# williamleif/GraphSAGE

Measured on NVIDIA H100. Metric: seed_nodes_per_sec, higher is better.
Workload: dtype f32

## Files before the change

### graphsage_b200/csrc/maxpool_tc.cu

```cuda
#include "tc_common.cuh"

namespace gs {

constexpr int MP_KCOLS = 64;
constexpr int MP_IMG = 128 * 128;
constexpr int MP_MAX_KB = 10;
constexpr int MP_STAGES = 3;
constexpr int MP_THREADS = 256;

struct MpParams {
  const __nv_bfloat16* table;
  int64_t n_rows, pitch;
  int32_t K, kblocks;
  const int32_t* row_ids;
  int64_t row0;
  int64_t n_groups;
  int32_t k, G;
  int32_t n_slices;
  const unsigned char* wimg;
  const float* bias;
  int32_t pool_mean;
  float* out;
  int64_t ldo;
  const float* dhp;
  int64_t lddhp;
  unsigned char* dp;
  float* dbm_part;
};

__global__ void __launch_bounds__(256) maxpool_pack_kernel(const float* __restrict__ W, int64_t ldw, int K, int hidden,
                                                           int kblocks, unsigned char* __restrict__ img) {
  const int slice = blockIdx.x / kblocks, kb = blockIdx.x % kblocks;
  unsigned char* dst = img + ((int64_t)slice * kblocks + kb) * MP_IMG;
  for (int q = threadIdx.x; q < 128 * 8; q += blockDim.x) {
    const int c = q >> 7, n = q & 127;
    const int gn = slice * 128 + n, k0 = kb * MP_KCOLS + c * 8;
    __nv_bfloat162 h[4];
#pragma unroll
    for (int e = 0; e < 4; ++e) {
      float a = (gn < hidden && k0 + 2 * e < K) ? W[(int64_t)(k0 + 2 * e) * ldw + gn] : 0.f;
      float b = (gn < hidden && k0 + 2 * e + 1 < K) ? W[(int64_t)(k0 + 2 * e + 1) * ldw + gn] : 0.f;
      h[e] = __floats2bfloat162_rn(a, b);
    }
    *reinterpret_cast<uint4*>(dst + sw128_off(n, c)) = *reinterpret_cast<uint4*>(h);
  }
}

template <bool kRowsA, int NT, int DEPTH, int PROD, bool kGrad = false>
__global__ void __launch_bounds__(MP_THREADS, NT == 128 ? 2 : 1) maxpool_mlp_kernel(const __grid_constant__ MpParams prm) {
  constexpr int ROWS_IMG = NT * 128;
  constexpr int STAGE = ROWS_IMG + MP_IMG;
  constexpr int CPT = NT / 32;
  constexpr int LOOK = MP_STAGES - DEPTH;
  constexpr int MI = kRowsA ? NT / 128 : 1;
  constexpr int NI = kRowsA ? 1 : NT / 128;
  constexpr int LD = NT + 1;
  static_assert(128 * LD * 4 <= MP_STAGES * STAGE, "epilogue staging must fit in the operand ring");
  static_assert(LOOK >= 1, "at least one K-block of prefetch");
  extern __shared__ unsigned char smem_raw[];
  __shared__ __align__(8) uint64_t full_b[MP_STAGES];
  unsigned char* smem = reinterpret_cast<unsigned char*>((reinterpret_cast<uintptr_t>(smem_raw) + 1023) & ~(uintptr_t)1023);
  const int tid = threadIdx.x, wg = tid >> 7, lane = tid & 31, wq = (tid >> 5) & 3;
  const int slice = blockIdx.x % prm.n_slices;
  const int64_t t = blockIdx.x / prm.n_slices;
  const int kblocks = prm.kblocks;

  if (tid == 0) {
    for (int s = 0; s < MP_STAGES; ++s) mbar_init(&full_b[s], 1);
    fence_mbar_init();
  }
  __syncthreads();

  const int c = tid & 7, r0 = tid >> 3;
  const int rows_valid = prm.G * prm.k;
  const __nv_bfloat16* rowp[CPT];
#pragma unroll
  for (int i = 0; i < CPT; ++i) {
    const int r = r0 + 32 * i;
    const int64_t flat = t * rows_valid + r;
    rowp[i] = nullptr;
    if (r < rows_valid && flat < prm.n_groups * prm.k) {
      int64_t id = prm.row_ids ? (int64_t)prm.row_ids[flat] : prm.row0 + flat;
      if (id < 0 || id >= prm.n_rows) id = prm.n_rows - 1;
      rowp[i] = prm.table + id * prm.pitch;
    }
  }
  const unsigned char* wsrc = prm.wimg + (int64_t)slice * kblocks * MP_IMG;
  auto stage_of = [&](int kb) { return smem + (size_t)(kb % MP_STAGES) * STAGE; };
  auto issue = [&](int kb) {
    if (kb < kblocks) {
      unsigned char* st = stage_of(kb);
      if (tid == 0) {
        mbar_expect_tx(&full_b[kb % MP_STAGES], MP_IMG);
        bulk_g2s(st + ROWS_IMG, wsrc + (int64_t)kb * MP_IMG, MP_IMG, &full_b[kb % MP_STAGES]);
      }
      if constexpr (PROD == 0) {
        const int col = kb * MP_KCOLS + c * 8;
#pragma unroll
        for (int i = 0; i < CPT; ++i) {
          int nbytes = 0;
          if (rowp[i] != nullptr && col < prm.K) nbytes = min(8, prm.K - col) * 2;
          const void* src = nbytes ? (const void*)(rowp[i] + col) : (const void*)prm.table;
          cp_async16(st + sw128_off(r0 + 32 * i, c), src, nbytes);
        }
      }
    }
    if constexpr (PROD == 0) cp_async_commit();
  };
  uint4 regs[PROD == 1 ? CPT : 1];
  auto load_regs = [&](int kb) {
    const int col = kb * MP_KCOLS + c * 8;
#pragma unroll
    for (int i = 0; i < CPT; ++i) {
      regs[i] = make_uint4(0, 0, 0, 0);
      if (rowp[i] == nullptr || col >= prm.K) continue;
      if (col + 8 <= prm.K) {
        regs[i] = __ldg(reinterpret_cast<const uint4*>(rowp[i] + col));
      } else {
        unsigned short h[8] = {0, 0, 0, 0, 0, 0, 0, 0};
        const unsigned short* src = reinterpret_cast<const unsigned short*>(rowp[i] + col);
        for (int e = 0; e < prm.K - col; ++e) h[e] = __ldg(src + e);
        regs[i] = *reinterpret_cast<const uint4*>(h);
      }
    }
  };

  for (int j = 0; j < LOOK; ++j) issue(j);
  if constexpr (PROD == 1) load_regs(0);
  float acc[MI * NI][64];
#pragma unroll
  for (int a = 0; a < MI * NI; ++a)
#pragma unroll
    for (int i = 0; i < 64; ++i) acc[a][i] = 0.f;
  for (int kb = 0; kb < kblocks; ++kb) {
    unsigned char* st = stage_of(kb);
    if constexpr (PROD == 0) {
      cp_async_wait<LOOK - 1>();
    } else {
#pragma unroll
      for (int i = 0; i < CPT; ++i) *reinterpret_cast<uint4*>(st + sw128_off(r0 + 32 * i, c)) = regs[i];
    }
    fence_proxy_async();
    __syncthreads();
    issue(kb + LOOK);
    if constexpr (PROD == 1) {
      if (kb + 1 < kblocks) load_regs(kb + 1);
    }
    mbar_wait(&full_b[kb % MP_STAGES], (uint32_t)(kb / MP_STAGES) & 1u);
    const uint32_t rows_s = smem_u32(st), w_s = smem_u32(st + ROWS_IMG);
#pragma unroll
    for (int a = 0; a < MI * NI; ++a) acc_fence(acc[a]);
    wgmma_fence();
#pragma unroll
    for (int k = 0; k < 4; ++k)
#pragma unroll
      for (int mi = 0; mi < MI; ++mi)
#pragma unroll
        for (int ni = 0; ni < NI; ++ni) {
          const uint64_t adesc = kRowsA ? make_smem_desc(rows_s + (uint32_t)((wg * (NT / 2) + mi * 64) * 128))
                                        : make_smem_desc(w_s + (uint32_t)(wg * 64 * 128));
          const uint64_t bdesc = kRowsA ? make_smem_desc(w_s) : make_smem_desc(rows_s + (uint32_t)(ni * 128 * 128));
          wgmma_m64n128<true>(acc[mi * NI + ni], adesc + (uint64_t)(k * 2), bdesc + (uint64_t)(k * 2),
                              (kb > 0 || k > 0) ? 1u : 0u);
        }
    wgmma_commit();
    wgmma_wait<DEPTH - 1>();
#pragma unroll
    for (int a = 0; a < MI * NI; ++a) acc_fence(acc[a]);
  }
  wgmma_wait<0>();
#pragma unroll
  for (int a = 0; a < MI * NI; ++a) acc_fence(acc[a]);
  if constexpr (PROD == 0) cp_async_wait<0>();
  __syncthreads();

  float* stage = reinterpret_cast<float*>(smem);
#pragma unroll
  for (int mi = 0; mi < MI; ++mi)
#pragma unroll
    for (int ni = 0; ni < NI; ++ni)
#pragma unroll
      for (int j = 0; j < 16; ++j)
#pragma unroll
        for (int e = 0; e < 4; ++e) {
          const int m = wq * 16 + (lane >> 2) + 8 * (e >> 1);
          const int n = 8 * j + 2 * (lane & 3) + (e & 1);
          const int row = kRowsA ? wg * (NT / 2) + mi * 64 + m : ni * 128 + n;
          const int col = kRowsA ? n : wg * 64 + m;
          stage[col * LD + row] = acc[mi * NI + ni][4 * j + e];
        }
  __syncthreads();
  const int k = prm.k, G = prm.G;
  if constexpr (kGrad) {
    static_assert(kRowsA && NT == 128, "B1 reads the <rows as A, 128-row tile> staging layout");
    const int cc = tid & (TC_BN - 1), hcol = slice * 128 + cc;
    const float b = prm.bias ? prm.bias[hcol] : 0.f;
    float part = 0.f;
    for (int g = tid >> 7; g < G; g += 2) {
      const int64_t gg = t * G + g;
      if (gg >= prm.n_groups) break;
      float* p = stage + cc * LD + g * k;
      const float d = prm.dhp[gg * prm.lddhp + hcol];
      float s = 0.f;
      if (prm.pool_mean) {
        const float q = d / (float)k;
        for (int j = 0; j < k; ++j) {
          const float v = (p[j] + b > 0.f) ? q : 0.f;
          p[j] = v;
          s += v;
        }
      } else {
        float m = -3.0e38f;
        for (int j = 0; j < k; ++j) m = fmaxf(m, p[j]);
        const float hp = fmaxf(m + b, 0.f);
        int cnt = 0;
        if (hp > 0.f)
          for (int j = 0; j < k; ++j) cnt += (p[j] + b == hp) ? 1 : 0;
        const float q = cnt ? d / (float)cnt : 0.f;
        for (int j = 0; j < k; ++j) {
          const float v = (cnt && p[j] + b == hp) ? q : 0.f;
          p[j] = v;
          s += v;
        }
      }
      part += s;
    }
    float* red = stage + TC_BN * LD;
    red[(tid >> 7) * TC_BN + cc] = part;
    __syncthreads();
    if (tid < TC_BN) prm.dbm_part[t * (int64_t)prm.n_slices * 128 + hcol] = red[cc] + red[TC_BN + cc];
    const int nvalid = (int)min((int64_t)G * k, prm.n_groups * k - t * (int64_t)G * k);
    unsigned char* img = prm.dp + (t * prm.n_slices + slice) * (int64_t)(2 * MP_IMG);
#pragma unroll
    for (int i = 0; i < (2 * 128 * 8) / MP_THREADS; ++i) {
      const int q = tid + MP_THREADS * i;
      const int h = q >> 10, n = (q >> 3) & 127, c = q & 7;
      const int r0 = h * 64 + c * 8;
      __nv_bfloat162 v[4];
#pragma unroll
      for (int e = 0; e < 4; ++e) {
        const float a0 = (r0 + 2 * e < nvalid) ? stage[n * LD + r0 + 2 * e] : 0.f;
        const float a1 = (r0 + 2 * e + 1 < nvalid) ? stage[n * LD + r0 + 2 * e + 1] : 0.f;
        v[e] = __floats2bfloat162_rn(a0, a1);
      }
      *reinterpret_cast<uint4*>(img + h * MP_IMG + sw128_off(n, c)) = *reinterpret_cast<uint4*>(v);
    }
  } else {
    for (int u = tid; u < TC_BN * G; u += MP_THREADS) {
      const int cc = u & (TC_BN - 1), g = u / TC_BN;
      const int64_t gg = t * G + g;
      if (gg >= prm.n_groups) break;
      const float* p = stage + cc * LD + g * k;
      const int hcol = slice * 128 + cc;
      const float b = prm.bias ? prm.bias[hcol] : 0.f;
      float res;
      if (prm.pool_mean) {
        float sacc = 0.f;
        for (int j = 0; j < k; ++j) sacc += fmaxf(p[j] + b, 0.f);
        res = sacc / (float)k;
      } else {
        float m = -3.0e38f;
        int j = 0;
        for (; j + 8 <= k; j += 8) {
          float v[8];
#pragma unroll
          for (int w = 0; w < 8; ++w) v[w] = p[j + w];
          m = fmaxf(m, fmaxf(fmaxf(fmaxf(v[0], v[1]), fmaxf(v[2], v[3])), fmaxf(fmaxf(v[4], v[5]), fmaxf(v[6], v[7]))));
        }
        for (; j < k; ++j) m = fmaxf(m, p[j]);
        res = fmaxf(m + b, 0.f);
      }
      prm.out[gg * prm.ldo + hcol] = res;
    }
  }
}

template <bool kRowsA, int NT, int DEPTH, int PROD>
static int32_t launch_k4(const MpParams& prm, int64_t n_tiles, int cluster, cudaStream_t st) {
  const void* fn = (const void*)maxpool_mlp_kernel<kRowsA, NT, DEPTH, PROD>;
  const int smem = MP_STAGES * (NT * 128 + MP_IMG) + 1024;
  const int32_t rc_attr = ensure_dyn_smem(fn, smem);
  if (rc_attr != GS_OK) return rc_attr;
  cudaLaunchConfig_t cfg;
  memset(&cfg, 0, sizeof(cfg));
  cfg.gridDim = dim3((unsigned)(n_tiles * prm.n_slices));
  cfg.blockDim = dim3((unsigned)MP_THREADS);
  cfg.dynamicSmemBytes = smem;
  cfg.stream = st;
  cudaLaunchAttribute attr;
  if (cluster > 1) {
    attr.id = cudaLaunchAttributeClusterDimension;
    attr.val.clusterDim.x = (unsigned)cluster;
    attr.val.clusterDim.y = 1;
    attr.val.clusterDim.z = 1;
    cfg.attrs = &attr;
    cfg.numAttrs = 1;
  }
  MpParams p = prm;
  void* args[1] = {(void*)&p};
  GS_CUDA(cudaLaunchKernelExC(&cfg, fn, args));
  return launch_check("maxpool_mlp_kernel");
}

template <bool kRowsA, int NT>
static int32_t launch_k4_by(const MpParams& prm, int64_t n_tiles, int cluster, int depth, int producer, cudaStream_t st) {
  if (depth == 2)
    return producer == 1 ? launch_k4<kRowsA, NT, 2, 1>(prm, n_tiles, cluster, st) : launch_k4<kRowsA, NT, 2, 0>(prm, n_tiles, cluster, st);
  return producer == 1 ? launch_k4<kRowsA, NT, 1, 1>(prm, n_tiles, cluster, st) : launch_k4<kRowsA, NT, 1, 0>(prm, n_tiles, cluster, st);
}

}

extern "C" {

int64_t gs_maxpool_mlp_workspace_bytes(int32_t K, int32_t hidden) {
  if (K < 1 || hidden < 1) return -1;
  const int kblocks = (K + gs::MP_KCOLS - 1) / gs::MP_KCOLS, slices = (hidden + 127) / 128;
  return (int64_t)kblocks * slices * gs::MP_IMG;
}

int32_t gs_maxpool_mlp_pack(const float* Wm, int64_t ldw, int32_t K, int32_t hidden, void* workspace, void* stream) {
  GS_REQUIRE(Wm && workspace && K >= 1 && hidden >= 1 && ldw >= hidden, "gs_maxpool_mlp_pack: bad arguments");
  GS_REQUIRE((reinterpret_cast<uintptr_t>(workspace) & 127u) == 0, "gs_maxpool_mlp_pack: workspace must be 128-byte aligned");
  const int kblocks = (K + gs::MP_KCOLS - 1) / gs::MP_KCOLS, slices = (hidden + 127) / 128;
  gs::maxpool_pack_kernel<<<kblocks * slices, 256, 0, (cudaStream_t)stream>>>(Wm, ldw, K, hidden, kblocks,
                                                                             (unsigned char*)workspace);
  return gs::launch_check("maxpool_pack_kernel");
}

static int32_t pool_mlp_fused(const void* table_bf16, int64_t n_rows, int32_t K, int64_t pitch, const int32_t* row_ids,
                              int64_t row0, int64_t n_groups, int32_t k, const void* packed_weights, const float* bias,
                              int32_t hidden, float* out, int64_t ldo, int32_t pool_mean, void* stream) {
  GS_REQUIRE(n_groups >= 0 && k >= 1, "gs_maxpool_mlp_fused: bad n_groups / k");
  if (n_groups == 0) return GS_OK;
  GS_REQUIRE(table_bf16 && packed_weights && out, "gs_maxpool_mlp_fused: NULL pointer");
  GS_REQUIRE(n_rows > 0 && n_rows < 0x7fffffffLL && K >= 1 && pitch >= K, "gs_maxpool_mlp_fused: bad table shape");
  GS_REQUIRE((pitch * 2) % 16 == 0 && (reinterpret_cast<uintptr_t>(table_bf16) & 15u) == 0,
             "gs_maxpool_mlp_fused: table rows must be 16-byte multiples and 16-byte aligned (pitch %% 8 == 0)");
  GS_REQUIRE((reinterpret_cast<uintptr_t>(packed_weights) & 127u) == 0, "gs_maxpool_mlp_fused: packed weights misaligned");
  const int nt = gs::tuning("k4_tile", 128) == 256 ? 256 : 128;
  if (k > nt || (K + gs::MP_KCOLS - 1) / gs::MP_KCOLS > gs::MP_MAX_KB || hidden % 128 != 0) {
    gs::set_error("gs_maxpool_mlp_fused: needs k <= %d, K <= %d, hidden %% 128 == 0 (k=%d K=%d hidden=%d)", nt,
                  gs::MP_MAX_KB * gs::MP_KCOLS, k, K, hidden);
    return GS_ERR_UNSUPPORTED;
  }
  GS_REQUIRE(ldo >= hidden, "gs_maxpool_mlp_fused: ldo < hidden");
  gs::MpParams prm;
  memset(&prm, 0, sizeof(prm));
  prm.table = (const __nv_bfloat16*)table_bf16;
  prm.n_rows = n_rows; prm.pitch = pitch; prm.K = K; prm.kblocks = (K + gs::MP_KCOLS - 1) / gs::MP_KCOLS;
  prm.row_ids = row_ids; prm.row0 = row0; prm.n_groups = n_groups; prm.k = k; prm.G = nt / k;
  prm.n_slices = hidden / 128;
  prm.wimg = (const unsigned char*)packed_weights; prm.bias = bias; prm.out = out; prm.ldo = ldo;
  prm.pool_mean = pool_mean;
  const int64_t n_tiles = (n_groups + prm.G - 1) / prm.G;
  GS_REQUIRE(n_tiles * prm.n_slices < 0x7fffffffLL, "gs_maxpool_mlp_fused: too many groups (%lld)", (long long)n_groups);
  int cluster = gs::tuning("k4_cluster", 0);
  if (cluster < 0 || cluster > prm.n_slices) cluster = prm.n_slices;
  while (cluster > 1 && (cluster > 8 || prm.n_slices % cluster != 0)) --cluster;
  const int depth = gs::tuning("k4_mma_depth", 1) == 2 ? 2 : 1;
  const int producer = gs::tuning("k4_producer", 0) == 1 ? 1 : 0;
  const bool rows_a = gs::tuning("k4_operands", 1) != 0;
  const cudaStream_t st = (cudaStream_t)stream;
  if (rows_a)
    return nt == 256 ? gs::launch_k4_by<true, 256>(prm, n_tiles, cluster, depth, producer, st)
                     : gs::launch_k4_by<true, 128>(prm, n_tiles, cluster, depth, producer, st);
  return nt == 256 ? gs::launch_k4_by<false, 256>(prm, n_tiles, cluster, depth, producer, st)
                   : gs::launch_k4_by<false, 128>(prm, n_tiles, cluster, depth, producer, st);
}

int32_t gs_maxpool_mlp_fused(const void* table_bf16, int64_t n_rows, int32_t K, int64_t pitch, const int32_t* row_ids,
                             int64_t row0, int64_t n_groups, int32_t k, const void* packed_weights, const float* bias,
                             int32_t hidden, float* out, int64_t ldo, void* stream) {
  return pool_mlp_fused(table_bf16, n_rows, K, pitch, row_ids, row0, n_groups, k, packed_weights, bias, hidden, out, ldo, 0,
                        stream);
}

int32_t gs_meanpool_mlp_fused(const void* table_bf16, int64_t n_rows, int32_t K, int64_t pitch, const int32_t* row_ids,
                              int64_t row0, int64_t n_groups, int32_t k, const void* packed_weights, const float* bias,
                              int32_t hidden, float* out, int64_t ldo, void* stream) {
  return pool_mlp_fused(table_bf16, n_rows, K, pitch, row_ids, row0, n_groups, k, packed_weights, bias, hidden, out, ldo, 1,
                        stream);
}

int64_t gs_pool_mlp_dp_bytes(int64_t n_groups, int32_t k, int32_t hidden) {
  if (n_groups < 0 || k < 1 || k > 128 || hidden < 128 || hidden % 128 != 0) return -1;
  const int64_t G = 128 / k, n_tiles = (n_groups + G - 1) / G;
  return n_tiles * hidden * (256 + 4);
}

int32_t gs_pool_mlp_backward_dp(const void* table_bf16, int64_t n_rows, int32_t K, int64_t pitch, const int32_t* row_ids,
                                int64_t row0, int64_t n_groups, int32_t k, const void* packed_weights, const float* bias,
                                int32_t hidden, const float* dhp, int64_t lddhp, int32_t pool_mean, void* dp, void* stream) {
  GS_REQUIRE(n_groups >= 0 && k >= 1, "gs_pool_mlp_backward_dp: bad n_groups / k");
  if (n_groups == 0) return GS_OK;
  GS_REQUIRE(table_bf16 && packed_weights && dhp && dp, "gs_pool_mlp_backward_dp: NULL pointer");
  GS_REQUIRE(n_rows > 0 && n_rows < 0x7fffffffLL && K >= 1 && pitch >= K, "gs_pool_mlp_backward_dp: bad table shape");
  GS_REQUIRE((pitch * 2) % 16 == 0 && (reinterpret_cast<uintptr_t>(table_bf16) & 15u) == 0,
             "gs_pool_mlp_backward_dp: table rows must be 16-byte multiples and 16-byte aligned (pitch %% 8 == 0)");
  GS_REQUIRE((reinterpret_cast<uintptr_t>(packed_weights) & 127u) == 0 && (reinterpret_cast<uintptr_t>(dp) & 15u) == 0,
             "gs_pool_mlp_backward_dp: packed weights / dp misaligned");
  if (k > 128 || (K + gs::MP_KCOLS - 1) / gs::MP_KCOLS > gs::MP_MAX_KB || hidden % 128 != 0 || hidden < 128) {
    gs::set_error("gs_pool_mlp_backward_dp: needs k <= 128, K <= %d, hidden %% 128 == 0 (k=%d K=%d hidden=%d)",
                  gs::MP_MAX_KB * gs::MP_KCOLS, k, K, hidden);
    return GS_ERR_UNSUPPORTED;
  }
  GS_REQUIRE(lddhp >= hidden, "gs_pool_mlp_backward_dp: lddhp < hidden");
  gs::MpParams prm;
  memset(&prm, 0, sizeof(prm));
  prm.table = (const __nv_bfloat16*)table_bf16;
  prm.n_rows = n_rows; prm.pitch = pitch; prm.K = K; prm.kblocks = (K + gs::MP_KCOLS - 1) / gs::MP_KCOLS;
  prm.row_ids = row_ids; prm.row0 = row0; prm.n_groups = n_groups; prm.k = k; prm.G = 128 / k;
  prm.n_slices = hidden / 128;
  prm.wimg = (const unsigned char*)packed_weights; prm.bias = bias; prm.pool_mean = pool_mean;
  prm.dhp = dhp; prm.lddhp = lddhp;
  const int64_t n_tiles = (n_groups + prm.G - 1) / prm.G;
  prm.dp = (unsigned char*)dp;
  prm.dbm_part = reinterpret_cast<float*>((unsigned char*)dp + n_tiles * hidden * 256);
  GS_REQUIRE(n_tiles * prm.n_slices < 0x7fffffffLL, "gs_pool_mlp_backward_dp: too many groups (%lld)", (long long)n_groups);
  const void* fn = (const void*)gs::maxpool_mlp_kernel<true, 128, 1, 0, true>;
  const int smem = gs::MP_STAGES * (128 * 128 + gs::MP_IMG) + 1024;
  const int32_t rc_attr = gs::ensure_dyn_smem(fn, smem);
  if (rc_attr != GS_OK) return rc_attr;
  gs::maxpool_mlp_kernel<true, 128, 1, 0, true>
      <<<(unsigned)(n_tiles * prm.n_slices), gs::MP_THREADS, smem, (cudaStream_t)stream>>>(prm);
  return gs::launch_check("maxpool_mlp_kernel<grad>");
}

}
```

Measured before the change: 3.432 million.

## Add warp-specialized persistent max-pool MLP kernel covering two hidden slices

```diff
diff --git a/graphsage_b200/csrc/maxpool_tc.cu b/graphsage_b200/csrc/maxpool_tc.cu
--- a/graphsage_b200/csrc/maxpool_tc.cu
+++ b/graphsage_b200/csrc/maxpool_tc.cu
@@ -46,6 +46,38 @@
   }
 }
 
+template <int NC>
+__device__ __forceinline__ void pool_store(const MpParams& prm, const float* stage, int ld, int64_t t, int col0, int tid,
+                                           int nthreads) {
+  const int k = prm.k, G = prm.G;
+  for (int u = tid; u < NC * G; u += nthreads) {
+    const int cc = u & (NC - 1), g = u / NC;
+    const int64_t gg = t * G + g;
+    if (gg >= prm.n_groups) break;
+    const float* p = stage + cc * ld + g * k;
+    const int hcol = col0 + cc;
+    const float b = prm.bias ? prm.bias[hcol] : 0.f;
+    float res;
+    if (prm.pool_mean) {
+      float sacc = 0.f;
+      for (int j = 0; j < k; ++j) sacc += fmaxf(p[j] + b, 0.f);
+      res = sacc / (float)k;
+    } else {
+      float m = -3.0e38f;
+      int j = 0;
+      for (; j + 8 <= k; j += 8) {
+        float v[8];
+#pragma unroll
+        for (int w = 0; w < 8; ++w) v[w] = p[j + w];
+        m = fmaxf(m, fmaxf(fmaxf(fmaxf(v[0], v[1]), fmaxf(v[2], v[3])), fmaxf(fmaxf(v[4], v[5]), fmaxf(v[6], v[7]))));
+      }
+      for (; j < k; ++j) m = fmaxf(m, p[j]);
+      res = fmaxf(m + b, 0.f);
+    }
+    prm.out[gg * prm.ldo + hcol] = res;
+  }
+}
+
 template <bool kRowsA, int NT, int DEPTH, int PROD, bool kGrad = false>
 __global__ void __launch_bounds__(MP_THREADS, NT == 128 ? 2 : 1) maxpool_mlp_kernel(const __grid_constant__ MpParams prm) {
   constexpr int ROWS_IMG = NT * 128;
@@ -246,32 +278,7 @@
       *reinterpret_cast<uint4*>(img + h * MP_IMG + sw128_off(n, c)) = *reinterpret_cast<uint4*>(v);
     }
   } else {
-    for (int u = tid; u < TC_BN * G; u += MP_THREADS) {
-      const int cc = u & (TC_BN - 1), g = u / TC_BN;
-      const int64_t gg = t * G + g;
-      if (gg >= prm.n_groups) break;
-      const float* p = stage + cc * LD + g * k;
-      const int hcol = slice * 128 + cc;
-      const float b = prm.bias ? prm.bias[hcol] : 0.f;
-      float res;
-      if (prm.pool_mean) {
-        float sacc = 0.f;
-        for (int j = 0; j < k; ++j) sacc += fmaxf(p[j] + b, 0.f);
-        res = sacc / (float)k;
-      } else {
-        float m = -3.0e38f;
-        int j = 0;
-        for (; j + 8 <= k; j += 8) {
-          float v[8];
-#pragma unroll
-          for (int w = 0; w < 8; ++w) v[w] = p[j + w];
-          m = fmaxf(m, fmaxf(fmaxf(fmaxf(v[0], v[1]), fmaxf(v[2], v[3])), fmaxf(fmaxf(v[4], v[5]), fmaxf(v[6], v[7]))));
-        }
-        for (; j < k; ++j) m = fmaxf(m, p[j]);
-        res = fmaxf(m + b, 0.f);
-      }
-      prm.out[gg * prm.ldo + hcol] = res;
-    }
+    pool_store<TC_BN>(prm, stage, LD, t, slice * 128, tid, MP_THREADS);
   }
 }
 
@@ -309,6 +316,162 @@
   return producer == 1 ? launch_k4<kRowsA, NT, 1, 1>(prm, n_tiles, cluster, st) : launch_k4<kRowsA, NT, 1, 0>(prm, n_tiles, cluster, st);
 }
 
+constexpr int MPP_THREADS = 384;
+constexpr int MPP_STAGES = 4;
+constexpr int MPP_STAGE = 3 * MP_IMG;
+constexpr int MPP_LD = 129;
+constexpr int MPP_SMEM = MPP_STAGES * MPP_STAGE + 64 * MPP_LD * 4 + 1024;
+
+template <uint32_t N>
+__device__ __forceinline__ void setmaxnreg_inc() { asm volatile("setmaxnreg.inc.sync.aligned.u32 %0;" ::"n"(N)); }
+template <uint32_t N>
+__device__ __forceinline__ void setmaxnreg_dec() { asm volatile("setmaxnreg.dec.sync.aligned.u32 %0;" ::"n"(N)); }
+__device__ __forceinline__ void cp_async_mbar_arrive(uint64_t* bar) {
+  asm volatile("cp.async.mbarrier.arrive.noinc.shared::cta.b64 [%0];" ::"r"(smem_u32(bar)) : "memory");
+}
+__device__ __forceinline__ void consumer_bar_sync() { asm volatile("bar.sync 1, 256;" ::: "memory"); }
+
+__global__ void __launch_bounds__(MPP_THREADS, 1) maxpool_mlp_persistent_kernel(const __grid_constant__ MpParams prm,
+                                                                                  int64_t n_units) {
+  extern __shared__ unsigned char smem_raw[];
+  __shared__ __align__(8) uint64_t full_b[MPP_STAGES], empty_b[MPP_STAGES];
+  unsigned char* smem = reinterpret_cast<unsigned char*>((reinterpret_cast<uintptr_t>(smem_raw) + 1023) & ~(uintptr_t)1023);
+  float* stage = reinterpret_cast<float*>(smem + MPP_STAGES * MPP_STAGE);
+  const int tid = threadIdx.x, wg = tid >> 7;
+  const int kblocks = prm.kblocks, n_pairs = (prm.n_slices + 1) >> 1;
+
+  if (tid == 0) {
+    for (int s = 0; s < MPP_STAGES; ++s) {
+      mbar_init(&full_b[s], 128 + 1);
+      mbar_init(&empty_b[s], 8);
+    }
+    fence_mbar_init();
+  }
+  __syncthreads();
+
+  if (wg == 0) {
+    setmaxnreg_dec<40>();
+    const int c = tid & 7, r0 = tid >> 3;
+    const int rows_valid = prm.G * prm.k;
+    uint32_t it = 0;
+    for (int64_t u = blockIdx.x; u < n_units; u += gridDim.x) {
+      const int64_t t = u / n_pairs;
+      const int s0 = 2 * (int)(u - t * n_pairs);
+      const bool two = s0 + 1 < prm.n_slices;
+      int32_t rid[8];
+#pragma unroll
+      for (int i = 0; i < 8; ++i) {
+        const int r = r0 + 16 * i;
+        const int64_t flat = t * rows_valid + r;
+        rid[i] = -1;
+        if (r < rows_valid && flat < prm.n_groups * prm.k) {
+          int64_t id = prm.row_ids ? (int64_t)prm.row_ids[flat] : prm.row0 + flat;
+          if (id < 0 || id >= prm.n_rows) id = prm.n_rows - 1;
+          rid[i] = (int32_t)id;
+        }
+      }
+      const unsigned char* wsrc = prm.wimg + (int64_t)s0 * kblocks * MP_IMG;
+      for (int kb = 0; kb < kblocks; ++kb, ++it) {
+        const int s = it % MPP_STAGES;
+        unsigned char* st = smem + s * MPP_STAGE;
+        mbar_wait(&empty_b[s], ((it / MPP_STAGES) & 1u) ^ 1u);
+        if (tid == 0) {
+          mbar_expect_tx(&full_b[s], two ? 2 * MP_IMG : MP_IMG);
+          bulk_g2s(st + MP_IMG, wsrc + (int64_t)kb * MP_IMG, MP_IMG, &full_b[s]);
+          if (two) bulk_g2s(st + 2 * MP_IMG, wsrc + (int64_t)(kblocks + kb) * MP_IMG, MP_IMG, &full_b[s]);
+        }
+        const int col = kb * MP_KCOLS + c * 8;
+#pragma unroll
+        for (int i = 0; i < 8; ++i) {
+          const int nbytes = (rid[i] >= 0 && col < prm.K) ? min(8, prm.K - col) * 2 : 0;
+          const void* src = nbytes ? (const void*)(prm.table + (int64_t)rid[i] * prm.pitch + col) : (const void*)prm.table;
+          cp_async16(st + sw128_off(r0 + 16 * i, c), src, nbytes);
+        }
+        cp_async_mbar_arrive(&full_b[s]);
+      }
+    }
+    cp_async_wait<0>();
+    return;
+  }
+
+  setmaxnreg_inc<232>();
+  const int cw = wg - 1, ctid = tid - 128, lane = tid & 31, wq = (tid >> 5) & 3;
+  float acc[2][64];
+#pragma unroll
+  for (int h = 0; h < 2; ++h)
+#pragma unroll
+    for (int i = 0; i < 64; ++i) acc[h][i] = 0.f;
+  uint32_t it = 0;
+  for (int64_t u = blockIdx.x; u < n_units; u += gridDim.x) {
+    const int64_t t = u / n_pairs;
+    const int s0 = 2 * (int)(u - t * n_pairs);
+    const bool two = s0 + 1 < prm.n_slices;
+    for (int kb = 0; kb < kblocks; ++kb, ++it) {
+      const int s = it % MPP_STAGES;
+      mbar_wait(&full_b[s], (it / MPP_STAGES) & 1u);
+      fence_proxy_async();
+      const uint32_t st = smem_u32(smem + s * MPP_STAGE);
+      const uint64_t adesc = make_smem_desc(st + (uint32_t)(cw * 64 * 128));
+      const uint64_t bdesc0 = make_smem_desc(st + MP_IMG), bdesc1 = make_smem_desc(st + 2 * MP_IMG);
+      acc_fence(acc[0]);
+      acc_fence(acc[1]);
+      if (two) {
+        wgmma_fence();
+#pragma unroll
+        for (int k = 0; k < 4; ++k) {
+          const uint32_t scale = (kb > 0 || k > 0) ? 1u : 0u;
+          wgmma_m64n128<true>(acc[0], adesc + (uint64_t)(k * 2), bdesc0 + (uint64_t)(k * 2), scale);
+          wgmma_m64n128<true>(acc[1], adesc + (uint64_t)(k * 2), bdesc1 + (uint64_t)(k * 2), scale);
+        }
+        wgmma_commit();
+      } else {
+        wgmma_fence();
+#pragma unroll
+        for (int k = 0; k < 4; ++k)
+          wgmma_m64n128<true>(acc[0], adesc + (uint64_t)(k * 2), bdesc0 + (uint64_t)(k * 2), (kb > 0 || k > 0) ? 1u : 0u);
+        wgmma_commit();
+      }
+      wgmma_wait<1>();
+      acc_fence(acc[0]);
+      acc_fence(acc[1]);
+      if (kb > 0 && lane == 0) mbar_arrive(&empty_b[(it - 1) % MPP_STAGES]);
+    }
+    wgmma_wait<0>();
+    acc_fence(acc[0]);
+    acc_fence(acc[1]);
+    if (lane == 0) mbar_arrive(&empty_b[(it - 1) % MPP_STAGES]);
+
+#pragma unroll
+    for (int h = 0; h < 2; ++h) {
+      if (h == 1 && !two) break;
+#pragma unroll
+      for (int q = 0; q < 2; ++q) {
+        consumer_bar_sync();
+#pragma unroll
+        for (int j = 8 * q; j < 8 * q + 8; ++j)
+#pragma unroll
+          for (int e = 0; e < 4; ++e) {
+            const int row = cw * 64 + wq * 16 + (lane >> 2) + 8 * (e >> 1);
+            const int col = 8 * (j - 8 * q) + 2 * (lane & 3) + (e & 1);
+            stage[col * MPP_LD + row] = acc[h][4 * j + e];
+          }
+        consumer_bar_sync();
+        pool_store<64>(prm, stage, MPP_LD, t, (s0 + h) * 128 + 64 * q, ctid, 256);
+      }
+    }
+  }
+}
+
+static int32_t launch_k4_persistent(const MpParams& prm, int64_t n_tiles, cudaStream_t st) {
+  const void* fn = (const void*)maxpool_mlp_persistent_kernel;
+  const int32_t rc_attr = ensure_dyn_smem(fn, MPP_SMEM);
+  if (rc_attr != GS_OK) return rc_attr;
+  const int64_t n_units = n_tiles * ((prm.n_slices + 1) / 2);
+  const unsigned grid = (unsigned)(n_units < sm_count() ? n_units : sm_count());
+  maxpool_mlp_persistent_kernel<<<grid, MPP_THREADS, MPP_SMEM, st>>>(prm, n_units);
+  return launch_check("maxpool_mlp_persistent_kernel");
+}
+
 }
 
 extern "C" {
@@ -356,12 +519,16 @@
   const int64_t n_tiles = (n_groups + prm.G - 1) / prm.G;
   GS_REQUIRE(n_tiles * prm.n_slices < 0x7fffffffLL, "gs_maxpool_mlp_fused: too many groups (%lld)", (long long)n_groups);
   int cluster = gs::tuning("k4_cluster", 0);
+  const bool default_cluster = cluster == 0;
   if (cluster < 0 || cluster > prm.n_slices) cluster = prm.n_slices;
   while (cluster > 1 && (cluster > 8 || prm.n_slices % cluster != 0)) --cluster;
   const int depth = gs::tuning("k4_mma_depth", 1) == 2 ? 2 : 1;
   const int producer = gs::tuning("k4_producer", 0) == 1 ? 1 : 0;
   const bool rows_a = gs::tuning("k4_operands", 1) != 0;
   const cudaStream_t st = (cudaStream_t)stream;
+  if (rows_a && nt == 128 && depth == 1 && producer == 0 && default_cluster &&
+      n_tiles * ((prm.n_slices + 1) / 2) >= gs::sm_count())
+    return gs::launch_k4_persistent(prm, n_tiles, st);
   if (rows_a)
     return nt == 256 ? gs::launch_k4_by<true, 256>(prm, n_tiles, cluster, depth, producer, st)
                      : gs::launch_k4_by<true, 128>(prm, n_tiles, cluster, depth, producer, st);
```

New measurement: 3.461 million, median of 6. No clear change (+0.8%).
